# SyamVangara/multigrid-petsc

Hardware: AMD Instinct MI355X
Metric: fp64 DOF-updates/sec per V-cycle at 1024^3 (higher is better)
Workload: dtype f64

## Files before the change

include/mgk.h:

```cpp
#ifndef MGK_H
#define MGK_H
#include <stddef.h>
#ifdef __cplusplus
extern "C" {
#endif

#define MGK_XOFF 16
#define MGK_EINVAL  10001
#define MGK_ENOGPU  10002
#define MGK_ECOMM   10003

typedef struct mgk_ctx mgk_ctx;

typedef struct mgk_geom {
    int  dim;
    int  nx, ny, nz;
    int  pitch;
    long plane;
    long org;
    long total;
} mgk_geom;

int  mgk_geom_init(mgk_geom *g, int dim, int nx, int ny, int nz);

// ... 348 lines not shown
    MGK_TUNE_J2_REG_PRED       = 36,
    MGK_TUNE_J2_RING_PRED      = 37,
    MGK_TUNE_PJ2D_WAVES        = 38,
    MGK_TUNE_J2_RING_OLD       = 39,
    MGK_TUNE_SRR_TY2           = 40,
    MGK_TUNE_SRR_TY4           = 41,
    MGK_TUNE_J2_ZERO_RINGB     = 45,
    MGK_TUNE_PJ2_COPY          = 46,
    MGK_TUNE_J3_2D_MARCH       = 50,
    MGK_TUNE_J3_2D_CHUNK4      = 51,
    MGK_TUNE_J3_2D_CHUNK8      = 52,
    MGK_TUNE_DISPATCH_ORDER    = 53,
    MGK_TUNE_XCD_ORDER         = 54,
    MGK_TUNE_RR2D_MARCH        = 55,
    MGK_TUNE_RR2D_SHORT        = 56,
    MGK_TUNE_RESERVED_57       = 57,
    MGK_TUNE_J3_2D_ODD_DOWN    = 58,
    MGK_TUNE_J3_2D_ALL_DOWN    = 59,
    MGK_TUNE_J3_2D_STORE_PLAIN = 60,
    MGK_TUNE_J3_2D_STORE_NT    = 61,
    MGK_TUNE_J3_3D_TY2         = 62,
    MGK_TUNE_J3_3D_TY3         = 63,
    MGK_TUNE_J3_3D_ROWWISE     = 64,
    MGK_TUNE_NO_EXACT_FMA      = 65
};

void mgk_set_tuning(int variant, int zchunk);

#ifdef __cplusplus
}
#endif
#endif
```

include/mgsolve.h:

```cpp
#ifndef MGSOLVE_H
#define MGSOLVE_H
#include "mgk.h"
#ifdef __cplusplus
extern "C" {
#endif

typedef enum { MG_KSP_RICHARDSON = 0, MG_KSP_CHEBYSHEV = 1 } mg_ksp_type;
typedef enum { MG_PREC_FP64 = 0, MG_PREC_MIXED = 1 } mg_precision;
typedef enum { MG_PC_JACOBI = 0, MG_PC_LINE_Y = 1, MG_PC_LINE_X = 2, MG_PC_LINE_ALT = 3, MG_PC_RBGS = 4 } mg_pc_type;

typedef enum mg_fuse_bits {
    MG_FUSE_RESNORM = 1,
    MG_FUSE_PROLONG_SWEEP = 2,
    MG_FUSE_RES_RESTRICT = 4,
    MG_FUSE_NORM_SWEEP = 8,
    MG_FUSE_MIXED_CORRECT = 16,
    MG_FUSE_PAIRS = 32,
    MG_FUSE_RES_RESTRICT_SMALL = 128,
    MG_FUSE_COARSE_ZERO_SWEEP = 256,
    MG_FUSE_LDS_TAIL = 512,
    MG_FUSE_SWEEP_RESTRICT = 1024,
    MG_FUSE_ZERO_TRIPLE = 2048,
    MG_FUSE_PROLONG_PAIR = 4096,
    MG_FUSE_TRIPLE_2D = 8192,
    MG_FUSE_PROLONG_PAIR_SLAB = 16384,
    MG_FUSE_CHEBY = 32768,
    MG_FUSE_DEFAULT = MG_FUSE_RESNORM | MG_FUSE_PROLONG_SWEEP | MG_FUSE_RES_RESTRICT | MG_FUSE_NORM_SWEEP | MG_FUSE_MIXED_CORRECT | MG_FUSE_PAIRS |
                      MG_FUSE_COARSE_ZERO_SWEEP | MG_FUSE_LDS_TAIL | MG_FUSE_SWEEP_RESTRICT | MG_FUSE_ZERO_TRIPLE | MG_FUSE_PROLONG_PAIR |
                      MG_FUSE_TRIPLE_2D | MG_FUSE_PROLONG_PAIR_SLAB | MG_FUSE_CHEBY
} mg_fuse_bits;

typedef struct mg_config {
    int dim;
    int npts;
    int levels;
    int v[2];
    int maxiter;
    int ksp_type;
    double scale;
    double emin, emax;
    double rtol;
    int device;
    int precision;
    int rank, nranks;
    int dist_min_n;
    int fuse;
    int overlap;
    int graph;
    int pair_min_n;
    int slab_chunk;
    int mesh;
    int pc_type;
    int line_tail;
// ... 54 lines not shown
```

multigrid_petsc_amd/__init__.py:

```python
from ._lib import load_mgk, load_mgpetsc, LibraryMissing
from .solver import Fuse
from .mgk import Tune, tuning
```

multigrid_petsc_amd/csrc/mg_solver.c:

```c
#include "mgsolve.h"
#include "mg_comm.h"
#include "mg_solver_internal.h"
#include <math.h>
#include <stdio.h>
#include <stdlib.h>
#include <string.h>
#include <time.h>

#define MG_PI 3.14159265358979323846
static __thread char g_mgerr[512] = "ok";
const char *mg_last_error(void) { return g_mgerr; }
static int mgfail(int code, const char *what) {
    snprintf(g_mgerr, sizeof(g_mgerr), "%s (code %d; kernel layer: %s)", what, code, mgk_last_error());
    return code;
}

typedef struct mg_ops {
    int esz;
    int (*jacobi_range)(mgk_ctx *, const mgk_geom *, const double *, double, double, const void *, const void *, void *, int, int, void *);
    int (*jacobi_zero)(mgk_ctx *, const mgk_geom *, double, double, const void *, void *, void *);
    int (*residual)(mgk_ctx *, const mgk_geom *, const double *, const void *, const void *, void *, void *);
    int (*restrict_fw)(mgk_ctx *, const mgk_geom *, const mgk_geom *, const void *, void *, void *);
    int (*prolong_add)(mgk_ctx *, const mgk_geom *, const mgk_geom *, const void *, void *, void *);
    int (*prolong_jacobi)(mgk_ctx *, const mgk_geom *, const mgk_geom *, const double *, double, double, const void *, const void *, const void *, void *, void *);
// ... 277 lines not shown
        return mgfail(MGK_EINVAL, "mg_solver_create: this build has no one-launch tail of the line cycles (mg_line_tail.c is not linked)");
    if (cfg->precision == MG_PREC_MIXED && (cfg->dim != 3 || cfg->ksp_type != MG_KSP_RICHARDSON))
        return mgfail(MGK_EINVAL, "mg_solver_create: mixed precision is built for 3-D, Richardson+Jacobi");
    for (int l = 0; l < cfg->levels; l++) {
        int n = mg_grid_n(cfg->npts, l);
        int f = 1 << l;
        if (n < 1 || (cfg->npts - 1) % f != 0 || (n & 1) == 0)
            return mgfail(MGK_EINVAL, "mg_solver_create: npts-1 must be 2^m with m >= levels (vertex-centred coarsening, src/matbuild.c:62-66)");
    }
    if (cfg->mesh != 0 && (cfg->mesh < 0 || cfg->mesh > 2 || cfg->dim != 2 || cfg->precision != MG_PREC_FP64 || cfg->nranks > 1))
        return mgfail(MGK_EINVAL, "mg_solver_create: -mesh 1/2 is built for 2-D, fp64, one GPU");
    if (cfg->nranks > 1 && (!comm || cfg->dim != 3))
        return mgfail(MGK_EINVAL, "mg_solver_create: nranks > 1 needs a communicator and dim == 3");
    if (cfg->ksp_type == MG_KSP_CHEBYSHEV && !(cfg->emax > cfg->emin && cfg->emin > 0.0))
        return mgfail(MGK_EINVAL, "mg_solver_create: chebyshev needs 0 < emin < emax (-ksp_chebyshev_eigenvalues)");

    mg_solver *s = (mg_solver *)calloc(1, sizeof(mg_solver));
    s->cfg = *cfg;
    if (s->cfg.rtol <= 0) s->cfg.rtol = 1.e-7;
    if (s->cfg.dist_min_n <= 0) {
        const int n0 = mg_grid_n(cfg->npts, 0);
        s->cfg.dist_min_n = n0 < 255 ? n0 : 255;
    }
    if (s->cfg.fuse < 0) s->cfg.fuse = MG_FUSE_DEFAULT;
    if (s->cfg.pair_min_n <= 0) s->cfg.pair_min_n = (cfg->dim == 3) ? 255 : 2047;
    if (s->cfg.pc_type == MG_PC_RBGS) s->cfg.fuse &= ~(MG_FUSE_POINT_JACOBI_PASSES & ~MG_FUSE_PROLONG_SWEEP);
    else if (s->cfg.pc_type != MG_PC_JACOBI) s->cfg.fuse &= ~MG_FUSE_POINT_JACOBI_PASSES;
    if (s->cfg.mesh) s->cfg.fuse &= ~MG_FUSE_NO_ROW_TABLE_FORM;
    if (s->cfg.overlap < 0) s->cfg.overlap = 1;
    if (s->cfg.graph < 0) s->cfg.graph = 1;
    if (s->cfg.nranks < 1) s->cfg.nranks = 1;
    s->comm = comm;
    s->levels = cfg->levels;
    int rc = mgk_ctx_create(&s->ctx, cfg->device);
    if (rc) { free(s); return mgfail(rc, "mg_solver_create: mgk_ctx_create"); }
    if (s->cfg.slab_chunk < 0) {
        const char *e = getenv("MG_SLAB_CHUNK");
        const int quarter = (mg_grid_n(cfg->npts, 0) / (s->cfg.nranks > 0 ? s->cfg.nranks : 1)) / 4;
        s->cfg.slab_chunk = (e && *e && atoi(e) >= 0) ? atoi(e) : (quarter > 32 ? quarter : 32);
    }
    if (s->cfg.nranks > 1 && s->cfg.dim == 3) mgk_ctx_set_chunk_planes(s->ctx, s->cfg.slab_chunk);

    s->ldist = 0;
    if (s->cfg.nranks > 1) {
        for (int l = 0; l < s->levels; l++) {
            int n = mg_grid_n(cfg->npts, l);
            if (n >= s->cfg.dist_min_n && n >= 2 * s->cfg.nranks) s->ldist = l + 1; else break;
// ... 606 lines not shown
        gc.nz = c1 - c0;
        CHK(O->prolong_add(s->ctx, &F->g, &gc, (char *)Cq->u + (size_t)O->esz * (size_t)c0 * (size_t)Cq->g.plane, F->u, NULL));
    } else {
        CHK(ensure_u_ghosts(s, P, Lc));
        CHK(O->prolong_add(s->ctx, &F->g, &Cq->g, Cq->u, F->u, NULL));
    }
    F->u_ghost_ok = 0;
    return 0;
}

static int pjp_ok(const mg_solver *s, int P) {
    const mg_level *L = &s->L[0];
    const int need = MG_FUSE_PROLONG_PAIR | MG_FUSE_SWEEP_RESTRICT | MG_FUSE_PAIRS | MG_FUSE_NORM_SWEEP | MG_FUSE_PROLONG_SWEEP | MG_FUSE_RESNORM;
    if ((s->cfg.fuse & need) != need || P != 0 || s->cfg.dim != 3 || s->cfg.mesh || s->cfg.ksp_type != MG_KSP_RICHARDSON) return 0;
    if (s->cfg.v[0] != 3 || s->levels < 2 || s->lgraph == 1 || L->n < s->cfg.pair_min_n || s->last_cycle) return 0;
    if (L->distributed) {
        const mg_level *Lc = &s->L[1];
        const int hi = s->cfg.rank < s->cfg.nranks - 1;
        if (!(s->cfg.fuse & MG_FUSE_PROLONG_PAIR_SLAB) || !Lc->distributed || !L->f[0].far || !Lc->f[0].far || L->nz_min < 8 || Lc->nz_min < 4) return 0;
        return mgk_prolong_jacobi2_slab_ok_f64(&L->f[0].g, &Lc->f[0].g, hi) && mgk_jacobi2_sumsq_ok_f64(&L->f[0].g);
    }
    return mgk_prolong_jacobi2_ok_f64(&L->f[0].g, &s->L[1].f[0].g) && mgk_jacobi2_sumsq_ok_f64(&L->f[0].g);
}
static int finalize_iterate(mg_solver *s) {
    if (!s->iterate_behind) return 0;
    mg_level *L = &s->L[0];
    mg_fset *F = &L->f[0];
    if (L->distributed) {
        CHK(ensure_u_ghosts(s, 0, L));
        CHK(mgk_jacobi_range_f64(s->ctx, &F->g, L->coef, L->dinv, s->cfg.scale, (const double *)F->b, (const double *)F->u, (double *)F->tmp, 0, F->g.nz, NULL));
    } else
    CHK(mgk_jacobi_f64(s->ctx, &F->g, L->coef, L->dinv, s->cfg.scale, (const double *)F->b, (const double *)F->u, (double *)F->tmp, NULL));
    swap_ptr(&F->u, &F->tmp);
    mgi_u_rewritten(F);
    s->iterate_behind = 0; s->spec_valid = 0;
    return 0;
}

static int prolong_smooth(mg_solver *s, int P, int l) {
    mg_level *Lf = &s->L[l], *Lc = &s->L[l + 1];
    mg_fset *F = &Lf->f[P], *Cq = &Lc->f[P];
    const mg_ops *O = &OPS[P];
    const int v0 = s->cfg.v[0];
    if (!(s->cfg.fuse & MG_FUSE_PROLONG_SWEEP) || (s->cfg.ksp_type != MG_KSP_RICHARDSON && !j3_2d_ok(s, P, l, v0)) || v0 < 1) {
        CHK(prolong_from(s, P, l));
        return smooth(s, P, l, v0, 0);
// ... 22 lines not shown
            Cq->b_ghost_ok = cb;
            CHK(rcx);
        }
        CHK(group_exchange(s, P, F, 0));
        const int zi0 = lo ? 4 : 0, zi1 = hi ? nz - 2 : nz;
        const int split = s->cfg.overlap && zi1 - zi0 >= 2;
#define PJ2S(z0, z1) mgk_prolong_jacobi2_slab_f64(s->ctx, &F->g, &Cq->g, &F->gfar, &Cq->gfar, Lf->coef, Lf->dinv, s->cfg.scale, (const double *)F->b, \
                        (const double *)Cq->u, (const double *)F->u, (double *)F->tmp, (const double *)F->far, (const double *)Cq->far, lo, hi, z0, z1, cs)
        if (split) CHK(PJ2S(zi0, zi1));
        CHK(mgk_stream_wait(s->ctx, cs, ms));
        Cq->u_ghost_pending = 0; Cq->u_ghost_ok = 1;
        F->u_ghost_pending = 0; F->u_ghost_ok = 1; F->b_ghost_ok = 1;
        if (split) {
            if (lo) CHK(PJ2S(0, 4));
            if (hi) CHK(PJ2S(nz - 2, nz));
        } else CHK(PJ2S(0, nz));
#undef PJ2S
        swap_ptr(&F->u, &F->tmp);
        mgi_u_rewritten(F);
        s->sweep_owed = 1;
        return 0;
    }
    if (l == 0 && pjp_ok(s, P)) {
        CHK(mgk_prolong_jacobi2_f64(s->ctx, &F->g, &Cq->g, Lf->coef, Lf->dinv, s->cfg.scale, (const double *)F->b, (const double *)Cq->u,
                                    (const double *)F->u, (double *)F->tmp, NULL));
        swap_ptr(&F->u, &F->tmp);
        mgi_u_rewritten(F);
        s->sweep_owed = 1;
        return 0;
    }
    mgk_geom gc = Cq->g;
    const void *ucoarse = Cq->u;
    if (Lf->distributed && !Lc->distributed) {
        int c0 = s->zstart[s->cfg.rank], c1 = s->zstart[s->cfg.rank + 1];
        gc.nz = c1 - c0;
        ucoarse = (const char *)Cq->u + (size_t)O->esz * (size_t)c0 * (size_t)Cq->g.plane;
    } else if (Lc->distributed) {
        CHK(begin_u_ghosts(s, P, Lc));
    }
    if (Lf->distributed && s->cfg.overlap && Lf->nz_min >= 4 && s->cfg.dim == 3) {
        const int nz = F->g.nz;
        CHK(begin_u_ghosts(s, P, Lf));
        CHK(O->prolong_jacobi_range(s->ctx, &F->g, &gc, Lf->coef, Lf->dinv, s->cfg.scale, F->b, ucoarse, F->u, F->tmp, 2, nz - 1, NULL));
        if (Lc->distributed) CHK(ensure_u_ghosts(s, P, Lc));
        CHK(ensure_u_ghosts(s, P, Lf));
        CHK(O->prolong_jacobi_range(s->ctx, &F->g, &gc, Lf->coef, Lf->dinv, s->cfg.scale, F->b, ucoarse, F->u, F->tmp, 0, 2, NULL));
        CHK(O->prolong_jacobi_range(s->ctx, &F->g, &gc, Lf->coef, Lf->dinv, s->cfg.scale, F->b, ucoarse, F->u, F->tmp, nz - 1, nz, NULL));
    } else {
// ... 264 lines not shown
        if (s->sweep_owed && L->distributed) {
            const int nz = F->g.nz, lo = s->cfg.rank > 0, hi = s->cfg.rank < s->cfg.nranks - 1;
            void *cs = mgk_stream_compute(s->ctx), *ms = mgk_stream_comm(s->ctx);
            int n1 = 0, n2 = 0, n3 = 0;
            CHK(group_exchange(s, 0, F, 0));
#define J2M(z0, z1, off, np) mgk_jacobi2_sumsq_mid_slab_f64(s->ctx, &F->g, &F->gfar, L->coef, L->dinv, s->cfg.scale, (const double *)F->b, (const double *)F->u, \
                                (double *)F->tmp, (const double *)F->far, lo, hi, z0, z1, off, np, cs)
            const int split = s->cfg.overlap && nz >= 6;
            if (split) {
                void *t = prof_begin_kind(s, 0, 1);
                int rc2 = J2M(2, nz - 2, 0, &n1);
                prof_end(s, t);
                CHK(rc2);
            }
            CHK(mgk_stream_wait(s->ctx, cs, ms));
            F->u_ghost_pending = 0; F->u_ghost_ok = 1; F->b_ghost_ok = 1;
            if (split) { CHK(J2M(0, 2, n1, &n2)); CHK(J2M(nz - 2, nz, n1 + n2, &n3)); }
            else CHK(J2M(0, nz, 0, &n1));
#undef J2M
            CHK(mgk_partials_finish(s->ctx, n1 + n2 + n3, &ss, NULL));
            s->sweep_owed = 0; s->iterate_behind = 1; s->spec_valid = 1;
            goto norm_done;
        }
        if (s->sweep_owed) {
            void *t = prof_begin_kind(s, 0, 1);
            int rc2 = mgk_jacobi2_sumsq_mid_f64(s->ctx, &F->g, L->coef, L->dinv, s->cfg.scale, (const double *)F->b, (const double *)F->u,
                                                (double *)F->tmp, &ss, NULL);
            prof_end(s, t);
            CHK(rc2);
            s->sweep_owed = 0; s->iterate_behind = 1; s->spec_valid = 1;
            goto norm_done;
        }
        if (jnorm && L->distributed && s->cfg.dim == 3 && (s->cfg.fuse & MG_FUSE_SWEEP_RESTRICT) && (s->cfg.fuse & MG_FUSE_PAIRS) && F->far && L->nz_min >= 6 &&
            s->cfg.v[0] >= 2 && L->n >= s->cfg.pair_min_n && L->n + 1 <= 1024 && s->lgraph != 1 && mgk_jacobi2_sumsq_ok_f64(&F->g)) {
            const int nz = F->g.nz, lo = s->cfg.rank > 0, hi = s->cfg.rank < s->cfg.nranks - 1;
            void *cs = mgk_stream_compute(s->ctx), *ms = mgk_stream_comm(s->ctx);
            int n1 = 0, n2 = 0, n3 = 0;
            CHK(group_exchange(s, 0, F, 0));
#define J2N(z0, z1, off, np) mgk_jacobi2_sumsq_slab_f64(s->ctx, &F->g, &F->gfar, L->coef, L->dinv, s->cfg.scale, (const double *)F->b, (const double *)F->u, \
                                (double *)F->tmp, (const double *)F->far, lo, hi, z0, z1, off, np, cs)
            const int split = s->cfg.overlap && nz >= 6;
            if (split) CHK(J2N(2, nz - 2, 0, &n1));
            CHK(mgk_stream_wait(s->ctx, cs, ms));
            F->u_ghost_pending = 0; F->u_ghost_ok = 1; F->b_ghost_ok = 1;
            if (split) { CHK(J2N(0, 2, n1, &n2)); CHK(J2N(nz - 2, nz, n1 + n2, &n3)); }
            else CHK(J2N(0, nz, 0, &n1));
// ... 226 lines not shown
```

multigrid_petsc_amd/csrc/mg_solver_internal.h:

```cpp
#ifndef MG_SOLVER_INTERNAL_H
#define MG_SOLVER_INTERNAL_H
#include "mgsolve.h"
#include "mg_comm.h"
#include "mg_cheby_coefs.h"

#define MG_MAX_LEVELS 32
#define MG_MAX_TIMERS 4096

#define MG_FUSE_POINT_JACOBI_PASSES (MG_FUSE_PROLONG_SWEEP | MG_FUSE_NORM_SWEEP | MG_FUSE_PAIRS | MG_FUSE_COARSE_ZERO_SWEEP | MG_FUSE_LDS_TAIL | \
                                     MG_FUSE_SWEEP_RESTRICT | MG_FUSE_ZERO_TRIPLE | MG_FUSE_PROLONG_PAIR | MG_FUSE_TRIPLE_2D | \
                                     MG_FUSE_PROLONG_PAIR_SLAB | MG_FUSE_CHEBY)
#define MG_FUSE_NO_ROW_TABLE_FORM   (MG_FUSE_MIXED_CORRECT | MG_FUSE_RES_RESTRICT_SMALL)

typedef struct mg_fset {
    mgk_geom g;
    void *u, *b, *rv, *tmp;
    int guess_nonzero;
    int u_ghost_ok;
    int u_ghost_pending;
    int jz_ready;
    int last_sweep_pending;
    int b_ghost_ok;
    int pre_done;
    void *far;
    void *far2, *bfar;
    int bfar_ok;
    mgk_geom gfar;
} mg_fset;

static inline void mgi_u_rewritten(mg_fset *F) { F->u_ghost_ok = 0; F->u_ghost_pending = 0; }

typedef struct mg_level {
    int n;
    int z0, nzl;
// ... 39 lines not shown
    unsigned char timer_kind[MG_MAX_TIMERS];
    int prof_kind;
    int ntimers_created;
    void *gm_field[MGK_KRYLOV_MAX + 3];
    int gm_nfields, gm_restart;
    double *gm_hdev;
};

enum { MG_CHEBY_ZERO = 0, MG_CHEBY_PLAIN = 1, MG_CHEBY_PROLONG = 2, MG_CHEBY_NORM = 3 };
extern int mg_cheby_pass(mg_solver *s, int l, int kind, double *sumsq) __attribute__((weak));
extern int mg_cheby_tail(mg_solver *s) __attribute__((weak));

extern int mg_line_tables(mg_solver *s, int l, const double *ctab_host) __attribute__((weak));
extern int mg_line_smooth(mg_solver *s, int l, int maxit) __attribute__((weak));
extern int mg_xline_tables(mg_solver *s, int l, const double *ctab_host) __attribute__((weak));
extern int mg_xline_smooth(mg_solver *s, int l, int maxit) __attribute__((weak));
extern int mg_line_chunk_tables(mg_solver *s, int l, const double *ctab_host) __attribute__((weak));
extern int mg_line_chunk_smooth(mg_solver *s, int l, int maxit) __attribute__((weak));
extern int mg_xline_chunk_tables(mg_solver *s, int l, const double *ctab_host) __attribute__((weak));
extern int mg_xline_chunk_smooth(mg_solver *s, int l, int maxit) __attribute__((weak));
extern int mg_line_tail(mg_solver *s) __attribute__((weak));
extern int mg_rbgs_smooth(mg_solver *s, int l, int maxit) __attribute__((weak));
extern int mg_rbgs_prolong_smooth(mg_solver *s, int l, int maxit) __attribute__((weak));
long mg_xline_stride(int n, int uniform);
void mg_xline_factor(int n, int rows, const double *ctab, long gs, double *g);

int    mgi_fail(int code, const char *what);
#define CHK(call) do { int rc_ = (call); if (rc_) return mgi_fail(rc_, #call); } while (0)
int    mgi_upload(mg_solver *s, const double *h, size_t n, double **d);
double mgi_wall(void);
int    mgi_start(mg_solver *s);
int    mgi_smooth(mg_solver *s, int l, int maxit);
int    mgi_vcycle_rooted(mg_solver *s, int l);
int    mgi_vcycle_once(mg_solver *s);
int    mgi_iterate(mg_solver *s);
int    mgi_finalize(mg_solver *s);
int    mgi_apply_cycle(mg_solver *s);
#endif
```

multigrid_petsc_amd/csrc/mgk_sweep3.hip:

```cpp
#include "mgk_dev.hpp"
#include <type_traits>

struct J3dArgs {
    const double *u, *b, *uc;
    double *out;
    int nx, ny, nxc, nyc;
    long rs, crs;
    int ntx, yc, nwaves, xcd, bous, plainst;
    double a0, a2, a3, a4, a6, dinv, scale;
    double ch[6];
    const double *ctab, *dtab;
    double *partials;
    double *rout;
};
template <bool PRO, bool ZG, bool NORM, bool TAB, int YC, bool CHEB = false>
__global__ void __launch_bounds__(256) k_jacobi3_2d(const J3dArgs a) {
    using VT = V16<double>;
    constexpr bool ZU = PRO && ZG, ZS = ZG && !PRO;
    const int lane = threadIdx.x & 63;
    int bid = blockIdx.x;
    if (a.xcd) bid = (bid & 7) * (gridDim.x >> 3) + (bid >> 3);
    const int wid = __builtin_amdgcn_readfirstlane(bid * 4 + (threadIdx.x >> 6));
    const int tx = wid % a.ntx, cy = wid / a.ntx;
    const int yc = YC > 0 ? YC : a.yc;
// ... 462 lines not shown
        *norm_parts = (int)(4 * nblk);
    }
    if (g_variant == MGK_TUNE_J3_3D_ROWWISE) hipLaunchKernelGGL((k_jacobi3_3d<TY, NORM, 0, false>), dim3(nblk), dim3(256), 0, S(c, stream), a);
    else if (exact_fma7(ex_coef)) hipLaunchKernelGGL((k_jacobi3_3d<TY, NORM, 1, true>), dim3(nblk), dim3(256), 0, S(c, stream), a);
    else hipLaunchKernelGGL((k_jacobi3_3d<TY, NORM, 1, false>), dim3(nblk), dim3(256), 0, S(c, stream), a);
    HIPCHK(hipGetLastError());
    return 0;
}
template <bool NORM>
static int jacobi3_3d(mgk_ctx *c, const mgk_geom *g, const double *coef, double dinv, double scale, const double *b, const double *u, double *unew,
                      void *stream, int *norm_parts) {
    if (!c || !g || g->dim != 3 || !coef || !b || !u || !unew || u == unew || b == unew) return fail(MGK_EINVAL, "mgk_jacobi3_f64: bad arguments (3-D)");
    J33Args a; memset(&a, 0, sizeof(a));
    a.u = u + g->org; a.b = b + g->org; a.out = unew + g->org;
    a.nx = g->nx; a.ny = g->ny; a.nz = g->nz; a.rs = g->pitch; a.ms = g->plane;
    set_coef7(a, coef);
    a.dinv = dinv; a.scale = scale;
    const int ty = (g_variant == MGK_TUNE_J3_3D_TY2) ? 2 : (g_variant == MGK_TUNE_J3_3D_TY3 || NORM) ? 3 : 4;
    if (ty == 2) return jacobi3_3d_launch<2, NORM>(c, a, g, coef, norm_parts, stream);
    if (ty == 3) return jacobi3_3d_launch<3, NORM>(c, a, g, coef, norm_parts, stream);
    if constexpr (!NORM) return jacobi3_3d_launch<4, NORM>(c, a, g, coef, norm_parts, stream);
    else return fail(MGK_EINVAL, "mgk_jacobi3_sumsq_f64: tile height not built");
}
extern "C" int mgk_jacobi3_f64(mgk_ctx *c, const mgk_geom *g, const double *coef, double dinv, double scale,
                               const double *b, const double *u, double *unew, void *stream) {
    return jacobi3_3d<false>(c, g, coef, dinv, scale, b, u, unew, stream, nullptr);
}
extern "C" int mgk_jacobi3_sumsq_f64(mgk_ctx *c, const mgk_geom *g, const double *coef, double dinv, double scale,
                                     const double *b, const double *u, double *unew, double *sumsq_host, void *stream) {
    if (!sumsq_host) return fail(MGK_EINVAL, "mgk_jacobi3_sumsq_f64: bad arguments");
    int nparts = 0;
    int rc = jacobi3_3d<true>(c, g, coef, dinv, scale, b, u, unew, stream, &nparts);
    if (rc) return rc;
    return finish_to_host(c, nparts, 1, S(c, stream), sumsq_host);
}

extern "C" int mgk_ipc_alloc(mgk_ctx *c, size_t bytes, void **ptr, void *handle64) {
    if (!c || !ptr || !handle64 || !bytes) return fail(MGK_EINVAL, "mgk_ipc_alloc: bad arguments");
    HIPCHK(hipSetDevice(c->device));
    HIPCHK(hipExtMallocWithFlags(ptr, bytes, hipDeviceMallocFinegrained));
    HIPCHK(hipMemsetAsync(*ptr, 0, bytes, c->compute));
    HIPCHK(hipStreamSynchronize(c->compute));
    hipIpcMemHandle_t h;
    HIPCHK(hipIpcGetMemHandle(&h, *ptr));
    static_assert(sizeof(h) == MGK_IPC_HANDLE_BYTES, "handle size");
    memcpy(handle64, &h, sizeof(h));
    return 0;
}
extern "C" int mgk_ipc_open(mgk_ctx *c, const void *handle64, void **ptr) {
    if (!c || !ptr || !handle64) return fail(MGK_EINVAL, "mgk_ipc_open: bad arguments");
    HIPCHK(hipSetDevice(c->device));
    hipIpcMemHandle_t h;
    memcpy(&h, handle64, sizeof(h));
    HIPCHK(hipIpcOpenMemHandle(ptr, h, hipIpcMemLazyEnablePeerAccess));
    return 0;
// ... 88 lines not shown
```

multigrid_petsc_amd/mgk.py:

```python
import contextlib
import ctypes as C
import enum
import numpy as np
from ._lib import load_mgk

c_dp = C.POINTER(C.c_double)


class Geom(C.Structure):
    _fields_ = [("dim", C.c_int), ("nx", C.c_int), ("ny", C.c_int), ("nz", C.c_int),
                ("pitch", C.c_int), ("plane", C.c_long), ("org", C.c_long), ("total", C.c_long)]


class MgkError(RuntimeError):
    pass


class Tune(enum.IntEnum):
    DEFAULT = -1
    STORE_PLAIN = 0
    STORE_NT = 1
    LDS_TILE = 30
    ROW = 31
    ROW_PD2 = 32
# ... 4 lines not shown
    J2_RING_PRED = 37
    PJ2D_WAVES = 38
    J2_RING_OLD = 39
    SRR_TY2 = 40
    SRR_TY4 = 41
    J2_ZERO_RINGB = 45
    PJ2_COPY = 46
    J3_2D_MARCH = 50
    J3_2D_CHUNK4 = 51
    J3_2D_CHUNK8 = 52
    DISPATCH_ORDER = 53
    XCD_ORDER = 54
    RR2D_MARCH = 55
    RR2D_SHORT = 56
    RESERVED_57 = 57
    J3_2D_ODD_DOWN = 58
    J3_2D_ALL_DOWN = 59
    J3_2D_STORE_PLAIN = 60
    J3_2D_STORE_NT = 61
    J3_3D_TY2 = 62
    J3_3D_TY3 = 63
    J3_3D_ROWWISE = 64
    NO_EXACT_FMA = 65


@contextlib.contextmanager
def tuning(variant=-1, zchunk=-1):
    L = load_mgk()
    L.mgk_set_tuning.restype, L.mgk_set_tuning.argtypes = None, [C.c_int, C.c_int]
    L.mgk_set_tuning(int(variant), int(zchunk))
    try:
        yield
    finally:
        L.mgk_set_tuning(-1, -1)


def _sigs(L):
    vp, i, d, sz = C.c_void_p, C.c_int, C.c_double, C.c_size_t
    G = C.POINTER(Geom)
    S = {
        "mgk_geom_init": (i, [G, i, i, i, i]),
        "mgk_device_count": (i, []),
        "mgk_set_device": (i, [i]),
        "mgk_ctx_create": (i, [C.POINTER(vp), i]),
        "mgk_ctx_destroy": (None, [vp]),
        "mgk_last_error": (C.c_char_p, []),
# ... 81 lines not shown
        "mgk_prolong_jacobi_f64": (i, [vp, G, G, c_dp, d, d, vp, vp, vp, vp, vp]),
        "mgk_prolong_jacobi_f32": (i, [vp, G, G, c_dp, d, d, vp, vp, vp, vp, vp]),
        "mgk_prolong_jacobi_range_f64": (i, [vp, G, G, c_dp, d, d, vp, vp, vp, vp, i, i, vp]),
        "mgk_prolong_jacobi_range_f32": (i, [vp, G, G, c_dp, d, d, vp, vp, vp, vp, i, i, vp]),
        "mgk_residual_restrict_range_f64": (i, [vp, G, G, c_dp, vp, vp, vp, i, i, vp]),
        "mgk_residual_restrict_range_f32": (i, [vp, G, G, c_dp, vp, vp, vp, i, i, vp]),
        "mgk_residual_restrict_slab_f64": (i, [vp, G, G, G, c_dp, vp, vp, vp, i, vp, i, i, vp]),
        "mgk_residual_restrict_slab_f32": (i, [vp, G, G, G, c_dp, vp, vp, vp, i, vp, i, i, vp]),
        "mgk_residual_restrict_2d_f64": (i, [vp, G, G, c_dp, vp, vp, vp, vp, d, d, vp]),
        "mgk_sweep_residual_restrict_f64": (i, [vp, G, G, c_dp, d, d, vp, vp, vp, vp, vp, d, d, vp]),
        "mgk_sweep_residual_restrict_ok_f64": (i, [G, G]),
        "mgk_jacobi2_sumsq_f64": (i, [vp, G, c_dp, d, d, vp, vp, vp, C.POINTER(d), vp]),
        "mgk_jacobi2_sumsq_ok_f64": (i, [G]),
        "mgk_jacobi2_sumsq_mid_f64": (i, [vp, G, c_dp, d, d, vp, vp, vp, C.POINTER(d), vp]),
        "mgk_prolong_jacobi2_ok_f64": (i, [G, G]),
        "mgk_prolong_jacobi2_f64": (i, [vp, G, G, c_dp, d, d, vp, vp, vp, vp, vp]),
        "mgk_jacobi2_zero_ok_f64": (i, [G]),
        "mgk_jacobi2_zero_ok_f32": (i, [G]),
        "mgk_jacobi2_zero_f64": (i, [vp, G, c_dp, d, d, vp, vp, vp]),
        "mgk_jacobi2_zero_f32": (i, [vp, G, c_dp, d, d, vp, vp, vp]),
        "mgk_jacobi2_2d_sumsq_f64": (i, [vp, G, c_dp, d, d, vp, vp, vp, C.POINTER(d), vp]),
        "mgk_jacobi3_f64": (i, [vp, G, c_dp, d, d, vp, vp, vp, vp]),
        "mgk_jacobi3_sumsq_f64": (i, [vp, G, c_dp, d, d, vp, vp, vp, C.POINTER(d), vp]),
        "mgk_jacobi3_2d_f64": (i, [vp, G, c_dp, d, d, vp, vp, vp, vp, vp, vp]),
        "mgk_jacobi3_2d_sumsq_f64": (i, [vp, G, c_dp, d, d, vp, vp, vp, vp, vp, C.POINTER(d), vp]),
        "mgk_jacobi3_2d_zero_f64": (i, [vp, G, c_dp, d, d, vp, vp, vp, vp, vp]),
        "mgk_jacobi3_2d_sumsq_store_f64": (i, [vp, G, c_dp, d, d, vp, vp, vp, vp, vp, vp, C.POINTER(d), vp]),
        "mgk_prolong_jacobi3_2d_f64": (i, [vp, G, G, c_dp, d, d, vp, vp, vp, vp, vp, vp, vp]),
        "mgk_cheby3_2d_f64": (i, [vp, G, c_dp, d, c_dp, vp, vp, vp, vp, vp, vp]),
        "mgk_cheby3_2d_sumsq_f64": (i, [vp, G, c_dp, d, c_dp, vp, vp, vp, vp, vp, C.POINTER(d), vp]),
        "mgk_cheby3_2d_zero_f64": (i, [vp, G, c_dp, d, c_dp, vp, vp, vp, vp, vp]),
        "mgk_prolong_cheby3_2d_f64": (i, [vp, G, G, c_dp, d, c_dp, vp, vp, vp, vp, vp, vp, vp]),
        "mgk_tail_cycle_cheby_f64": (i, [vp, G, i, C.POINTER(i), c_dp, c_dp, C.POINTER(vp), C.POINTER(vp), d, d, i, i, vp, vp, vp]),
        "mgk_sweep_residual_restrict_2d_f64": (i, [vp, G, G, c_dp, d, d, vp, vp, vp, vp, vp, d, d, vp]),
        "mgk_jacobi2_sumsq_slab_f64": (i, [vp, G, G, c_dp, d, d, vp, vp, vp, vp, i, i, i, i, i, C.POINTER(i), vp]),
        "mgk_jacobi2_sumsq_mid_slab_f64": (i, [vp, G, G, c_dp, d, d, vp, vp, vp, vp, i, i, i, i, i, C.POINTER(i), vp]),
        "mgk_prolong_jacobi2_slab_ok_f64": (i, [G, G, i]),
        "mgk_prolong_jacobi2_slab_f64": (i, [vp, G, G, G, G, c_dp, d, d, vp, vp, vp, vp, vp, vp, i, i, i, i, vp]),
        "mgk_sweep_residual_restrict_slab_ok_f64": (i, [G, G]),
        "mgk_sweep_residual_restrict_slab_f64": (i, [vp, G, G, G, c_dp, d, d, vp, vp, vp, vp, vp, vp, i, i, vp, i, i, vp]),
        "mgk_ctx_set_chunk_planes": (i, [vp, i]),
        "mgk_residual_f64_to_f32_jz": (i, [vp, G, G, c_dp, vp, vp, vp, vp, d, d, C.POINTER(d), vp]),
        "mgk_correct_residual_f64_f32_jz": (i, [vp, G, G, c_dp, vp, vp, vp, vp, vp, vp, d, d, C.POINTER(d), vp]),
        "mgk_tail_cycle_f64": (i, [vp, G, i, C.POINTER(i), c_dp, c_dp, d, i, i, vp, vp, vp]),
        "mgk_tail_fmg_f64": (i, [vp, G, i, C.POINTER(i), c_dp, c_dp, d, i, i, i, vp, vp, vp]),
        "mgk_interp_jacobi2_ok_f64": (i, [G, G]),
# ... 150 lines not shown
```

multigrid_petsc_amd/solver.py:

```python
import ctypes as C
import enum

import numpy as np

from ._lib import load_mgpetsc


class MgConfig(C.Structure):
    _fields_ = [("dim", C.c_int), ("npts", C.c_int), ("levels", C.c_int), ("v", C.c_int * 2),
                ("maxiter", C.c_int), ("ksp_type", C.c_int), ("scale", C.c_double),
                ("emin", C.c_double), ("emax", C.c_double), ("rtol", C.c_double),
                ("device", C.c_int), ("precision", C.c_int), ("rank", C.c_int), ("nranks", C.c_int),
                ("dist_min_n", C.c_int), ("fuse", C.c_int), ("overlap", C.c_int), ("graph", C.c_int),
                ("pair_min_n", C.c_int), ("slab_chunk", C.c_int), ("mesh", C.c_int), ("pc_type", C.c_int),
                ("line_tail", C.c_int), ("xline_chunk", C.c_int), ("line_chunk", C.c_int)]


class MgError(RuntimeError):
    pass


class Fuse(enum.IntFlag):
    RESNORM = 1
    PROLONG_SWEEP = 2
    RES_RESTRICT = 4
    NORM_SWEEP = 8
    MIXED_CORRECT = 16
    PAIRS = 32
    RES_RESTRICT_SMALL = 128
    COARSE_ZERO_SWEEP = 256
    LDS_TAIL = 512
    SWEEP_RESTRICT = 1024
    ZERO_TRIPLE = 2048
    PROLONG_PAIR = 4096
    TRIPLE_2D = 8192
    PROLONG_PAIR_SLAB = 16384
    CHEBY = 32768
    DEFAULT = (RESNORM | PROLONG_SWEEP | RES_RESTRICT | NORM_SWEEP | MIXED_CORRECT | PAIRS | COARSE_ZERO_SWEEP | LDS_TAIL | SWEEP_RESTRICT |
               ZERO_TRIPLE | PROLONG_PAIR | TRIPLE_2D | PROLONG_PAIR_SLAB | CHEBY)


_KSP = {"richardson": 0, "chebyshev": 1}
_PC = {"jacobi": 0, "yline": 1, "xline": 2, "altline": 3}
_PC_GS = {"rbgs": 4}


def _lib():
    L = load_mgpetsc()
    if getattr(L, "_mg_sigs", False):
        return L
    vp, i, d = C.c_void_p, C.c_int, C.c_double
    L.mg_config_default.argtypes = [C.POINTER(MgConfig)]
    L.mg_solver_create.restype = i
    L.mg_solver_create.argtypes = [C.POINTER(vp), C.POINTER(MgConfig), vp]
    L.mg_solver_destroy.argtypes = [vp]
    L.mg_last_error.restype = C.c_char_p
    for f in ("mg_solver_set_rhs_problem", "mg_solver_reset", "mg_solver_solve", "mg_solver_sync"):
        getattr(L, f).restype = i
        getattr(L, f).argtypes = [vp]
    L.mg_solver_set_rhs_host.restype = i
    L.mg_solver_set_rhs_host.argtypes = [vp, vp]
    L.mg_solver_cycles.restype = i
# ... 201 lines not shown
```

Measured before the change: 389.3 billion.

## Add stacked three-sweep 3-D Jacobi kernel and fuse middle sweeps on finest level

Measured after the change: 418.3 billion (median of 6 runs). 7.4% higher.

```diff
diff --git a/include/mgk.h b/include/mgk.h
--- a/include/mgk.h
+++ b/include/mgk.h
@@ -394,7 +394,10 @@
     MGK_TUNE_J3_3D_TY2         = 62,
     MGK_TUNE_J3_3D_TY3         = 63,
     MGK_TUNE_J3_3D_ROWWISE     = 64,
-    MGK_TUNE_NO_EXACT_FMA      = 65
+    MGK_TUNE_NO_EXACT_FMA      = 65,
+    MGK_TUNE_J3_3D_WAVES       = 66,
+    MGK_TUNE_J3_3D_STACKED     = 67,
+    MGK_TUNE_J3_3D_STACKED_DISPATCH = 68
 };
 
 void mgk_set_tuning(int variant, int zchunk);
diff --git a/include/mgk_sweep3.h b/include/mgk_sweep3.h
--- /dev/null
+++ b/include/mgk_sweep3.h
@@ -0,0 +1,15 @@
+#ifndef MGK_SWEEP3_H
+#define MGK_SWEEP3_H
+#include "mgk.h"
+#ifdef __cplusplus
+extern "C" {
+#endif
+
+int  mgk_jacobi3_mid_ok_f64(const mgk_geom *g);
+int  mgk_jacobi3_sumsq_mid_f64(mgk_ctx *ctx, const mgk_geom *g, const double *coef, double dinv, double scale,
+                               const double *b, const double *u, double *unew, double *sumsq_host, void *stream);
+
+#ifdef __cplusplus
+}
+#endif
+#endif
diff --git a/include/mgsolve.h b/include/mgsolve.h
--- a/include/mgsolve.h
+++ b/include/mgsolve.h
@@ -29,6 +29,8 @@
                       MG_FUSE_COARSE_ZERO_SWEEP | MG_FUSE_LDS_TAIL | MG_FUSE_SWEEP_RESTRICT | MG_FUSE_ZERO_TRIPLE | MG_FUSE_PROLONG_PAIR |
                       MG_FUSE_TRIPLE_2D | MG_FUSE_PROLONG_PAIR_SLAB | MG_FUSE_CHEBY
 } mg_fuse_bits;
+#define MG_FUSE_TRIPLE_MID 65536
+#define MG_FUSE_AUTO (MG_FUSE_DEFAULT | MG_FUSE_TRIPLE_MID)
 
 typedef struct mg_config {
     int dim;
diff --git a/multigrid_petsc_amd/__init__.py b/multigrid_petsc_amd/__init__.py
--- a/multigrid_petsc_amd/__init__.py
+++ b/multigrid_petsc_amd/__init__.py
@@ -1,3 +1,3 @@
 from ._lib import load_mgk, load_mgpetsc, LibraryMissing
-from .solver import Fuse
+from .solver import Fuse, FUSE_AUTO, FUSE_TRIPLE_MID
 from .mgk import Tune, tuning
diff --git a/multigrid_petsc_amd/csrc/mg_solver.c b/multigrid_petsc_amd/csrc/mg_solver.c
--- a/multigrid_petsc_amd/csrc/mg_solver.c
+++ b/multigrid_petsc_amd/csrc/mg_solver.c
@@ -323,7 +323,7 @@
         const int n0 = mg_grid_n(cfg->npts, 0);
         s->cfg.dist_min_n = n0 < 255 ? n0 : 255;
     }
-    if (s->cfg.fuse < 0) s->cfg.fuse = MG_FUSE_DEFAULT;
+    if (s->cfg.fuse < 0) s->cfg.fuse = MG_FUSE_AUTO;
     if (s->cfg.pair_min_n <= 0) s->cfg.pair_min_n = (cfg->dim == 3) ? 255 : 2047;
     if (s->cfg.pc_type == MG_PC_RBGS) s->cfg.fuse &= ~(MG_FUSE_POINT_JACOBI_PASSES & ~MG_FUSE_PROLONG_SWEEP);
     else if (s->cfg.pc_type != MG_PC_JACOBI) s->cfg.fuse &= ~MG_FUSE_POINT_JACOBI_PASSES;
@@ -976,6 +976,11 @@
     }
     return mgk_prolong_jacobi2_ok_f64(&L->f[0].g, &s->L[1].f[0].g) && mgk_jacobi2_sumsq_ok_f64(&L->f[0].g);
 }
+static int triple_mid_ok(const mg_solver *s) {
+    if (!(s->cfg.fuse & MG_FUSE_TRIPLE_MID) || !mg_triple_mid_pass || !mg_triple_mid_fits) return 0;
+    if (s->cfg.nranks != 1 || s->L[0].distributed || s->cfg.v[0] != 3 || s->lgraph == 1) return 0;
+    return srr_ok(s, 0, 0) && mg_triple_mid_fits(s);
+}
 static int finalize_iterate(mg_solver *s) {
     if (!s->iterate_behind) return 0;
     mg_level *L = &s->L[0];
@@ -1044,8 +1049,11 @@
         return 0;
     }
     if (l == 0 && pjp_ok(s, P)) {
-        CHK(mgk_prolong_jacobi2_f64(s->ctx, &F->g, &Cq->g, Lf->coef, Lf->dinv, s->cfg.scale, (const double *)F->b, (const double *)Cq->u,
-                                    (const double *)F->u, (double *)F->tmp, NULL));
+        void *t = triple_mid_ok(s) ? prof_begin_kind(s, 0, 1) : NULL;
+        int rc2 = mgk_prolong_jacobi2_f64(s->ctx, &F->g, &Cq->g, Lf->coef, Lf->dinv, s->cfg.scale, (const double *)F->b, (const double *)Cq->u,
+                                          (const double *)F->u, (double *)F->tmp, NULL);
+        prof_end(s, t);
+        CHK(rc2);
         swap_ptr(&F->u, &F->tmp);
         mgi_u_rewritten(F);
         s->sweep_owed = 1;
@@ -1356,6 +1364,14 @@
             s->sweep_owed = 0; s->iterate_behind = 1; s->spec_valid = 1;
             goto norm_done;
         }
+        if (s->sweep_owed && triple_mid_ok(s)) {
+            void *t = prof_begin_kind(s, 0, 2);
+            int rc2 = mg_triple_mid_pass(s, &ss);
+            prof_end(s, t);
+            CHK(rc2);
+            s->sweep_owed = 0; s->iterate_behind = 1; s->spec_valid = 2;
+            goto norm_done;
+        }
         if (s->sweep_owed) {
             void *t = prof_begin_kind(s, 0, 1);
             int rc2 = mgk_jacobi2_sumsq_mid_f64(s->ctx, &F->g, L->coef, L->dinv, s->cfg.scale, (const double *)F->b, (const double *)F->u,
diff --git a/multigrid_petsc_amd/csrc/mg_solver_internal.h b/multigrid_petsc_amd/csrc/mg_solver_internal.h
--- a/multigrid_petsc_amd/csrc/mg_solver_internal.h
+++ b/multigrid_petsc_amd/csrc/mg_solver_internal.h
@@ -9,7 +9,7 @@
 
 #define MG_FUSE_POINT_JACOBI_PASSES (MG_FUSE_PROLONG_SWEEP | MG_FUSE_NORM_SWEEP | MG_FUSE_PAIRS | MG_FUSE_COARSE_ZERO_SWEEP | MG_FUSE_LDS_TAIL | \
                                      MG_FUSE_SWEEP_RESTRICT | MG_FUSE_ZERO_TRIPLE | MG_FUSE_PROLONG_PAIR | MG_FUSE_TRIPLE_2D | \
-                                     MG_FUSE_PROLONG_PAIR_SLAB | MG_FUSE_CHEBY)
+                                     MG_FUSE_PROLONG_PAIR_SLAB | MG_FUSE_CHEBY | MG_FUSE_TRIPLE_MID)
 #define MG_FUSE_NO_ROW_TABLE_FORM   (MG_FUSE_MIXED_CORRECT | MG_FUSE_RES_RESTRICT_SMALL)
 
 typedef struct mg_fset {
@@ -95,6 +95,8 @@
 extern int mg_line_tail(mg_solver *s) __attribute__((weak));
 extern int mg_rbgs_smooth(mg_solver *s, int l, int maxit) __attribute__((weak));
 extern int mg_rbgs_prolong_smooth(mg_solver *s, int l, int maxit) __attribute__((weak));
+extern int mg_triple_mid_fits(const mg_solver *s) __attribute__((weak));
+extern int mg_triple_mid_pass(mg_solver *s, double *sumsq) __attribute__((weak));
 long mg_xline_stride(int n, int uniform);
 void mg_xline_factor(int n, int rows, const double *ctab, long gs, double *g);
 
diff --git a/multigrid_petsc_amd/csrc/mg_triple.c b/multigrid_petsc_amd/csrc/mg_triple.c
--- /dev/null
+++ b/multigrid_petsc_amd/csrc/mg_triple.c
@@ -0,0 +1,16 @@
+#include "mg_solver_internal.h"
+#include "mgk_sweep3.h"
+#include <stddef.h>
+
+int mg_triple_mid_fits(const mg_solver *s) {
+    const mg_level *L = &s->L[0];
+    return s->cfg.dim == 3 && !L->distributed && mgk_jacobi3_mid_ok_f64(&L->f[0].g);
+}
+
+int mg_triple_mid_pass(mg_solver *s, double *sumsq) {
+    mg_level *L = &s->L[0];
+    mg_fset *F = &L->f[0];
+    CHK(mgk_jacobi3_sumsq_mid_f64(s->ctx, &F->g, L->coef, L->dinv, s->cfg.scale, (const double *)F->b, (const double *)F->u, (double *)F->tmp,
+                                  sumsq, NULL));
+    return 0;
+}
diff --git a/multigrid_petsc_amd/csrc/mgk_sweep3.hip b/multigrid_petsc_amd/csrc/mgk_sweep3.hip
--- a/multigrid_petsc_amd/csrc/mgk_sweep3.hip
+++ b/multigrid_petsc_amd/csrc/mgk_sweep3.hip
@@ -1,4 +1,5 @@
 #include "mgk_dev.hpp"
+#include "mgk_sweep3.h"
 #include <type_traits>
 
 struct J3dArgs {
@@ -508,15 +509,229 @@
     if constexpr (!NORM) return jacobi3_3d_launch<4, NORM>(c, a, g, coef, norm_parts, stream);
     else return fail(MGK_EINVAL, "mgk_jacobi3_sumsq_f64: tile height not built");
 }
+struct J3sArgs {
+    const double *u, *b;
+    double *out;
+    int nx, ny, nz;
+    long rs, ms;
+    int ntx, nty, ntz, zc, xcd;
+    double a0, a1, a2, a3, a4, a5, a6, dinv, scale;
+    double *partials;
+};
+#define J3S_WAVES 8
+#define J3S_ROWS 4
+template <int R, int NORM, bool EX>
+__global__ void __launch_bounds__(64 * J3S_WAVES) k_jacobi3s(const J3sArgs a) {
+    constexpr int NW = J3S_WAVES, Y = NW * R - 6;
+    constexpr unsigned XROW = 1024, XBUF = 3 * NW * 2 * XROW;
+    using VT = V16<double>;
+    __shared__ __attribute__((aligned(16))) char xch[2 * XBUF];
+    const int lane = threadIdx.x & 63;
+    const int w = __builtin_amdgcn_readfirstlane((int)(threadIdx.x >> 6));
+    int bid = blockIdx.x;
+    if (a.xcd) bid = (bid & 7) * (gridDim.x >> 3) + (bid >> 3);
+    const bool live = bid < a.ntx * a.nty * a.ntz;
+    const int tile = live ? bid : 0;
+    const int tx = tile % a.ntx, ty = (tile / a.ntx) % a.nty, tz = tile / (a.ntx * a.nty);
+    const int z0 = tz * a.zc, z1 = min(z0 + a.zc, a.nz);
+    const int t0 = z0 - 4, tend = live ? z1 : t0;
+    const int yb = ty * Y, yw = yb - 3 + w * R;
+    const int x0 = 2 * (tx * 60 + lane - 2);
+    const bool xin = (x0 >= 0 && x0 < a.nx);
+    const bool lastvec = (x0 + 2 > a.nx);
+    const bool store = (lane >= 2 && lane <= 61 && xin);
+    const unsigned lo = (unsigned)(8 * min(x0, a.nx + 1) + 32);
+    const char *__restrict__ ub_ = reinterpret_cast<const char *>(a.u) - 32;
+    const char *__restrict__ bb_ = reinterpret_cast<const char *>(a.b) - 32;
+    char *__restrict__ ob_ = reinterpret_cast<char *>(a.out) - 32;
+    long uro[R], bro[R];
+    unsigned long long rowm[R], rown[R];
+#pragma unroll
+    for (int q = 0; q < R; q++) {
+        const int y = yw + q;
+        uro[q] = 8 * (long)min(max(y, -1), a.ny) * a.rs;
+        bro[q] = 8 * (long)min(max(y, 0), a.ny - 1) * a.rs;
+        rowm[q] = (y >= 0 && y < a.ny) ? ~0ull : 0ull;
+        rown[q] = (y >= yb && y < yb + Y && y < a.ny) ? ~0ull : 0ull;
+    }
+    const unsigned long long Mx0 = xin ? ~0ull : 0ull, Mx1 = (xin && !lastvec) ? ~0ull : 0ull;
+    auto andm = [](double v, unsigned long long m) -> double { return __longlong_as_double((long long)((unsigned long long)__double_as_longlong(v) & m)); };
+    double nacc = 0.0;
+    const unsigned xl = (unsigned)lane * 16u;
+    const unsigned xw = (unsigned)(w * 2) * XROW + xl;
+    const unsigned xs = (unsigned)(max(w - 1, 0) * 2 + 1) * XROW + xl;
+    const unsigned xn = (unsigned)(min(w + 1, NW - 1) * 2) * XROW + xl;
+    auto xput = [&](unsigned buf, int f, const VT &first, const VT &last) {
+        char *p = xch + buf + (unsigned)f * (NW * 2 * XROW) + xw;
+        *reinterpret_cast<VT *>(p) = first;
+        *reinterpret_cast<VT *>(p + XROW) = last;
+    };
+    auto xget = [&](unsigned buf, int f, VT &south, VT &north) {
+        const char *p = xch + buf + (unsigned)f * (NW * 2 * XROW);
+        south = *reinterpret_cast<const VT *>(p + xs);
+        north = *reinterpret_cast<const VT *>(p + xn);
+    };
+    auto ldu = [&](VT (&P)[R], int z) {
+        const char *pz = ub_ + 8 * (long)min(max(z, -1), a.nz) * a.ms;
+#pragma unroll
+        for (int q = 0; q < R; q++) P[q] = *reinterpret_cast<const VT *>(pz + uro[q] + (size_t)lo);
+    };
+    auto ldb = [&](VT (&P)[R], int z) {
+        const char *pz = bb_ + 8 * (long)min(max(z, 0), a.nz - 1) * a.ms;
+#pragma unroll
+        for (int q = 0; q < R; q++) P[q] = ldv_stream(reinterpret_cast<const double *>(pz + bro[q] + (size_t)lo), true);
+    };
+    auto stage = [&](VT (&OUT)[R], const VT (&DN)[R], const VT &hs, const VT (&C)[R], const VT &hn, const VT (&UP)[R], const VT (&BB)[R],
+                     unsigned long long zm, auto maskrows, auto norm, unsigned long long nm) {
+        double s_[R][2];
+#pragma unroll
+        for (int q = 0; q < R; q++) { s_[q][0] = a.a0 * DN[q].v[0]; s_[q][1] = a.a0 * DN[q].v[1]; }
+#pragma unroll
+        for (int q = 0; q < R; q++) { const VT &sv = (q == 0) ? hs : C[q > 0 ? q - 1 : 0]; s_[q][0] = madd<EX>(s_[q][0], a.a1, sv.v[0]); s_[q][1] = madd<EX>(s_[q][1], a.a1, sv.v[1]); }
+#pragma unroll
+        for (int q = 0; q < R; q++) { s_[q][0] = madd<EX>(s_[q][0], a.a2, lane_up<true>(C[q].v[1])); s_[q][1] = madd<EX>(s_[q][1], a.a2, C[q].v[0]); }
+#pragma unroll
+        for (int q = 0; q < R; q++) { s_[q][0] = s_[q][0] + a.a3 * C[q].v[0]; s_[q][1] = s_[q][1] + a.a3 * C[q].v[1]; }
+#pragma unroll
+        for (int q = 0; q < R; q++) { s_[q][0] = madd<EX>(s_[q][0], a.a4, C[q].v[1]); s_[q][1] = madd<EX>(s_[q][1], a.a4, lane_dn<true>(C[q].v[0])); }
+#pragma unroll
+        for (int q = 0; q < R; q++) { const VT &nv = (q == R - 1) ? hn : C[q < R - 1 ? q + 1 : R - 1]; s_[q][0] = madd<EX>(s_[q][0], a.a5, nv.v[0]); s_[q][1] = madd<EX>(s_[q][1], a.a5, nv.v[1]); }
+#pragma unroll
+        for (int q = 0; q < R; q++) { s_[q][0] = madd<EX>(s_[q][0], a.a6, UP[q].v[0]); s_[q][1] = madd<EX>(s_[q][1], a.a6, UP[q].v[1]); }
+#pragma unroll
+        for (int q = 0; q < R; q++) {
+            const double r0 = BB[q].v[0] - s_[q][0], r1 = BB[q].v[1] - s_[q][1];
+            const double zz0 = r0 * a.dinv, zz1 = r1 * a.dinv;
+            const double v0 = C[q].v[0] + a.scale * zz0, v1 = C[q].v[1] + a.scale * zz1;
+            const unsigned long long mu = decltype(maskrows)::value ? (rowm[q] & zm) : ~0ull;
+            OUT[q].v[0] = andm(v0, Mx0 & mu); OUT[q].v[1] = andm(v1, Mx1 & mu);
+            if constexpr (decltype(norm)::value) {
+                const unsigned long long mn = rown[q] & nm;
+                const double n0 = andm(r0, mn), n1 = andm(r1, Mx1 & mn);
+                nacc += n0 * n0; nacc += n1 * n1;
+            }
+        }
+    };
+    using yes = std::true_type; using no = std::false_type;
+    const VT Z = v16_zero<double>();
+    VT U[3][R];
+    VT P[3][R];
+    VT Q[3][R];
+    VT B[3][R];
+    ldu(U[0], t0 + 1); ldu(U[1], t0 + 2); ldu(U[2], t0 + 3);
+    ldb(B[2], t0 + 2);
+#pragma unroll
+    for (int k = 0; k < 3; k++)
+#pragma unroll
+        for (int q = 0; q < R; q++) { P[k][q] = Z; Q[k][q] = Z; if (k < 2) B[k][q] = Z; }
+    xput(0, 0, U[1][0], U[1][R - 1]);
+    __syncthreads();
+    auto step = [&](auto phc, int t) {
+        constexpr int PH = decltype(phc)::value, S0 = PH % 3, S1 = (PH + 1) % 3, S2 = (PH + 2) % 3;
+        const unsigned rb = (unsigned)((t - t0) & 1) * XBUF, wb = XBUF - rb;
+        const unsigned long long z2m = (t + 2 >= 0 && t + 2 < a.nz) ? ~0ull : 0ull, z1m = (t + 1 >= 0 && t + 1 < a.nz) ? ~0ull : 0ull;
+        const unsigned long long z2own = (t + 2 >= z0 && t + 2 < z1) ? ~0ull : 0ull, z1own = (t + 1 >= z0 && t + 1 < z1) ? ~0ull : 0ull;
+        VT hs, hn;
+        xget(rb, 0, hs, hn);
+        stage(P[S2], U[S0], hs, U[S1], hn, U[S2], B[S2], z2m, yes{}, std::integral_constant<bool, NORM == 1>{}, z2own);
+        ldu(U[S0], t + 4);
+        if (t >= z0 - 2) {
+            xget(rb, 1, hs, hn);
+            stage(Q[S2], P[S0], hs, P[S1], hn, P[S2], B[S1], z1m, yes{}, std::integral_constant<bool, NORM == 2>{}, z1own);
+            if (t >= z0) {
+                VT O[R];
+                xget(rb, 2, hs, hn);
+                stage(O, Q[S0], hs, Q[S1], hn, Q[S2], B[S0], ~0ull, no{}, no{}, 0ull);
+                char *pz = ob_ + 8 * (long)t * a.ms;
+#pragma unroll
+                for (int q = 0; q < R; q++)
+                    if (store && rown[q]) stv_stream(reinterpret_cast<double *>(pz + bro[q] + (size_t)lo), O[q]);
+            }
+        }
+        ldb(B[S0], t + 3);
+        xput(wb, 0, U[S2][0], U[S2][R - 1]);
+        xput(wb, 1, P[S2][0], P[S2][R - 1]);
+        xput(wb, 2, Q[S2][0], Q[S2][R - 1]);
+        __syncthreads();
+    };
+    for (int t = t0; t < tend; t += 3) {
+        step(std::integral_constant<int, 0>{}, t);
+        if (t + 1 < tend) step(std::integral_constant<int, 1>{}, t + 1);
+        if (t + 2 < tend) step(std::integral_constant<int, 2>{}, t + 2);
+    }
+    if (NORM) {
+        const double sb = block_sum(store ? nacc : 0.0, reinterpret_cast<double *>(xch));
+        if (threadIdx.x == 0) a.partials[blockIdx.x] = sb;
+    }
+}
+static bool jacobi3s_shape_ok(const mgk_geom *g) { return g && g->dim == 3 && (g->nx + 1 == 512 || g->nx + 1 == 1024); }
+static int jacobi3s_takes(const mgk_geom *g) {
+    if (g_variant == MGK_TUNE_J3_3D_STACKED || g_variant == MGK_TUNE_J3_3D_STACKED_DISPATCH) return 1;
+    if (g_variant == MGK_TUNE_J3_3D_WAVES || g_variant == MGK_TUNE_J3_3D_TY2 || g_variant == MGK_TUNE_J3_3D_TY3 || g_variant == MGK_TUNE_J3_3D_ROWWISE ||
+        g_variant == MGK_TUNE_DISPATCH_ORDER) return 0;
+    return jacobi3s_shape_ok(g) ? 1 : 0;
+}
+template <int NORM>
+static int jacobi3s(mgk_ctx *c, const mgk_geom *g, const double *coef, double dinv, double scale, const double *b, const double *u, double *unew,
+                    void *stream, int *norm_parts, const char *who) {
+    static thread_local char msg[160];
+    if (!c || !g || g->dim != 3 || !coef || !b || !u || !unew || u == unew || b == unew) {
+        snprintf(msg, sizeof(msg), "%s: bad arguments (3-D; unew must not be u or b)", who);
+        return fail(MGK_EINVAL, msg);
+    }
+    if (!jacobi3s_shape_ok(g)) {
+        snprintf(msg, sizeof(msg), "%s: the stacked three-sweep pass is built for whole 3-D grids with rows of 512 or 1024 (nx = 511, 1023)", who);
+        return fail(MGK_EINVAL, msg);
+    }
+    constexpr int R = (NORM == 1) ? 3 : J3S_ROWS, Y = J3S_WAVES * R - 6;
+    J3sArgs a; memset(&a, 0, sizeof(a));
+    a.u = u + g->org; a.b = b + g->org; a.out = unew + g->org;
+    a.nx = g->nx; a.ny = g->ny; a.nz = g->nz; a.rs = g->pitch; a.ms = g->plane;
+    set_coef7(a, coef);
+    a.dinv = dinv; a.scale = scale;
+    a.ntx = ((g->nx + 1) / 2 + 59) / 60;
+    a.nty = (g->ny + Y - 1) / Y;
+    const long per = (long)a.ntx * a.nty;
+    long best = 1; double bestc = 0.0;
+    for (long n = 1; n <= 16 && g->nz / n >= 8; n++) {
+        const double cost = (double)((per * n + 255) / 256) * (double)((g->nz + n - 1) / n + 12);
+        if (n == 1 || cost < bestc) { best = n; bestc = cost; }
+    }
+    const Chunks ch = cut_chunks_n(c, g->nz, best, { 8,  true,  false,  true,  0, 0});
+    a.zc = ch.len; a.ntz = (int)ch.count;
+    unsigned nblk = (unsigned)(per * a.ntz);
+    a.xcd = (g_variant != MGK_TUNE_J3_3D_STACKED_DISPATCH && nblk >= 64) ? 1 : 0;
+    if (a.xcd) nblk = (nblk + 7u) & ~7u;
+    if (NORM) {
+        if (!norm_parts || (long)nblk > c->max_partials) { snprintf(msg, sizeof(msg), "%s: more blocks than partial slots", who); return fail(MGK_EINVAL, msg); }
+        a.partials = c->partials;
+        *norm_parts = (int)nblk;
+    }
+    if (exact_fma7(coef)) hipLaunchKernelGGL((k_jacobi3s<R, NORM, true>), dim3(nblk), dim3(64 * J3S_WAVES), 0, S(c, stream), a);
+    else hipLaunchKernelGGL((k_jacobi3s<R, NORM, false>), dim3(nblk), dim3(64 * J3S_WAVES), 0, S(c, stream), a);
+    HIPCHK(hipGetLastError());
+    return 0;
+}
 extern "C" int mgk_jacobi3_f64(mgk_ctx *c, const mgk_geom *g, const double *coef, double dinv, double scale,
                                const double *b, const double *u, double *unew, void *stream) {
+    if (jacobi3s_takes(g)) return jacobi3s<0>(c, g, coef, dinv, scale, b, u, unew, stream, nullptr, "mgk_jacobi3_f64");
     return jacobi3_3d<false>(c, g, coef, dinv, scale, b, u, unew, stream, nullptr);
+}
+extern "C" int mgk_jacobi3_mid_ok_f64(const mgk_geom *g) { return jacobi3s_shape_ok(g) ? 1 : 0; }
+extern "C" int mgk_jacobi3_sumsq_mid_f64(mgk_ctx *c, const mgk_geom *g, const double *coef, double dinv, double scale,
+                                         const double *b, const double *u, double *unew, double *sumsq_host, void *stream) {
+    if (!sumsq_host) return fail(MGK_EINVAL, "mgk_jacobi3_sumsq_mid_f64: bad arguments");
+    int nparts = 0;
+    int rc = jacobi3s<2>(c, g, coef, dinv, scale, b, u, unew, stream, &nparts, "mgk_jacobi3_sumsq_mid_f64");
+    if (rc) return rc;
+    return finish_to_host(c, nparts, 1, S(c, stream), sumsq_host);
 }
 extern "C" int mgk_jacobi3_sumsq_f64(mgk_ctx *c, const mgk_geom *g, const double *coef, double dinv, double scale,
                                      const double *b, const double *u, double *unew, double *sumsq_host, void *stream) {
     if (!sumsq_host) return fail(MGK_EINVAL, "mgk_jacobi3_sumsq_f64: bad arguments");
     int nparts = 0;
-    int rc = jacobi3_3d<true>(c, g, coef, dinv, scale, b, u, unew, stream, &nparts);
+    int rc = jacobi3s_takes(g) ? jacobi3s<1>(c, g, coef, dinv, scale, b, u, unew, stream, &nparts, "mgk_jacobi3_sumsq_f64")
+                               : jacobi3_3d<true>(c, g, coef, dinv, scale, b, u, unew, stream, &nparts);
     if (rc) return rc;
     return finish_to_host(c, nparts, 1, S(c, stream), sumsq_host);
 }
diff --git a/multigrid_petsc_amd/mgk.py b/multigrid_petsc_amd/mgk.py
--- a/multigrid_petsc_amd/mgk.py
+++ b/multigrid_petsc_amd/mgk.py
@@ -50,6 +50,9 @@
     J3_3D_TY3 = 63
     J3_3D_ROWWISE = 64
     NO_EXACT_FMA = 65
+    J3_3D_WAVES = 66
+    J3_3D_STACKED = 67
+    J3_3D_STACKED_DISPATCH = 68
 
 
 @contextlib.contextmanager
@@ -177,6 +180,8 @@
         "mgk_jacobi2_2d_sumsq_f64": (i, [vp, G, c_dp, d, d, vp, vp, vp, C.POINTER(d), vp]),
         "mgk_jacobi3_f64": (i, [vp, G, c_dp, d, d, vp, vp, vp, vp]),
         "mgk_jacobi3_sumsq_f64": (i, [vp, G, c_dp, d, d, vp, vp, vp, C.POINTER(d), vp]),
+        "mgk_jacobi3_sumsq_mid_f64": (i, [vp, G, c_dp, d, d, vp, vp, vp, C.POINTER(d), vp]),
+        "mgk_jacobi3_mid_ok_f64": (i, [G]),
         "mgk_jacobi3_2d_f64": (i, [vp, G, c_dp, d, d, vp, vp, vp, vp, vp, vp]),
         "mgk_jacobi3_2d_sumsq_f64": (i, [vp, G, c_dp, d, d, vp, vp, vp, vp, vp, C.POINTER(d), vp]),
         "mgk_jacobi3_2d_zero_f64": (i, [vp, G, c_dp, d, d, vp, vp, vp, vp, vp]),
diff --git a/multigrid_petsc_amd/solver.py b/multigrid_petsc_amd/solver.py
--- a/multigrid_petsc_amd/solver.py
+++ b/multigrid_petsc_amd/solver.py
@@ -38,6 +38,10 @@
     CHEBY = 32768
     DEFAULT = (RESNORM | PROLONG_SWEEP | RES_RESTRICT | NORM_SWEEP | MIXED_CORRECT | PAIRS | COARSE_ZERO_SWEEP | LDS_TAIL | SWEEP_RESTRICT |
                ZERO_TRIPLE | PROLONG_PAIR | TRIPLE_2D | PROLONG_PAIR_SLAB | CHEBY)
+
+
+FUSE_TRIPLE_MID = 65536
+FUSE_AUTO = int(Fuse.DEFAULT) | FUSE_TRIPLE_MID
 
 
 _KSP = {"richardson": 0, "chebyshev": 1}
```
